# pathint/RankCompV3.jl

Hardware: AMD Instinct MI355X
Metric: gene-pair·sample comparisons/sec at 20k genes × 1k samples (higher is better)
Workload: dtype u16

## Files before the change

rankcompv3.jl_amd/_ffi.py:

```python
from __future__ import annotations

import ctypes
import os
import subprocess
from typing import NamedTuple

import numpy as np

_HERE = os.path.dirname(os.path.abspath(__file__))
LIB_PATH = os.environ.get("REO_LIB_PATH") or os.path.join(_HERE, "libreo_hip.so")
CSRC = os.path.join(_HERE, "csrc")

REO_OK, REO_EINVAL, REO_EHIP, REO_ECOMM, REO_ENOMEM = 0, -1, -2, -3, -4
NTIMINGS = 12
CALL_BINS = 8192

SYMBOLS = [
    "reo_version", "reo_last_error", "reo_create", "reo_destroy", "reo_trim_memory", "reo_set_shard", "reo_set_allreduce", "reo_set_allgather",
    "reo_create_multi", "reo_comm_unique_id", "reo_comm_init_rank",
    "reo_set_matrix_f64", "reo_set_matrix_i64", "reo_set_matrix_dev_f64", "reo_set_matrix_dev_i64",
    "reo_set_matrix_f32", "reo_set_matrix_i32", "reo_set_matrix_dev_f32", "reo_set_matrix_dev_i32",
    "reo_set_matrix_rm_f64", "reo_set_matrix_rm_i64", "reo_set_matrix_rm_f32", "reo_set_matrix_rm_i32",
    "reo_set_matrix_csc_f64", "reo_set_matrix_csc_i64", "reo_set_matrix_csc_f32", "reo_set_matrix_csc_i32",
    "reo_set_groups", "reo_compute_thresholds", "reo_set_thresholds", "reo_get_thresholds", "reo_threshold",
# ... 1203 lines not shown

    def set_profiling(self, on: bool) -> None:
        check(self._L.reo_set_profiling(self._h, 1 if on else 0))

    def reset_timings(self) -> None:
        check(self._L.reo_reset_timings(self._h))

    def timings(self) -> dict:
        ms = np.zeros(NTIMINGS, dtype=np.float64)
        check(self._L.reo_get_timings(self._h, _ptr(ms), NTIMINGS))
        return {"transform_ms": ms[0], "k1_ms": ms[1], "k2_ms": ms[2], "iter_ms": ms[3], "k3_ms": max(ms[3] - ms[2], 0.0), "k2_launches": int(ms[4]),
                "k1_launches": int(ms[5]), "exchange_ms": ms[6], "pseudobulk_ms": ms[7], "k2_full_ms": ms[8],
                "k2_full_launches": int(ms[9]), "k2_delta_ms": ms[10], "set_matrix_host_wall_ms": ms[11]}

    def info(self) -> dict:
        w = np.zeros(42, dtype=np.int64)
        check(self._L.reo_get_info(self._h, _ptr(w), 42))
        v = np.zeros(28, dtype=np.int64)
        v[:] = w[:28]
        return {"G": int(v[0]), "S": int(v[1]), "Gp": int(v[2]), "table_bytes": int(v[3]), "has_ties": int(v[4]),
                "tiles_owned": int(v[5]), "tiles_total": int(v[6]), "tile_i": int(v[7]), "chunk_j": int(v[8]),
                "chunks_per_panel": int(v[9]), "unit_h": int(v[10]), "sample_slots": int(v[11]),
                "shared_group_counts": int(v[12]), "group_count_bytes": int(v[13]), "transform_in_lds": int(v[14]), "xcc_local_histograms": int(v[15]),
                "cycle_period": int(v[16]), "cycle_found_at_pass": int(v[17]), "cycle_passes_skipped": int(v[18]), "upload_link_bytes": int(v[19]),
                "eager_range_launches": int(v[20]), "rowmajor_upload": int(v[21]),
                "csc_upload": int(v[22]), "csc_nnz": int(v[23]), "resident_dtype": int(v[24]),
                "k1_slot_order": int(v[25]), "k1_half_tiles_separated": int(v[26]), "csc_device": int(v[27]),
                "k1_unslot_form": int(w[28]), "contrast_treat": int(w[29]), "k1_slot_sides": int(w[30]),
                "masked_build": int(w[31]), "k1_slot_slice": int(w[32]), "planes_on_demand": int(w[33]),
                "perm_batch": int(w[34]), "perm_kernel_us": int(w[35]),
                "top_pairs_hist_us": int(w[36]), "top_pairs_emit_us": int(w[37]),
                "top_pairs_null_batch": int(w[38]), "top_pairs_null_us": int(w[39]),
                "top_pairs_loo_words_us": int(w[40]), "top_pairs_loo_select_us": int(w[41])}
```

rankcompv3.jl_amd/csrc/api.hip:

```cpp
#include <execinfo.h>
#include <signal.h>
#include <unistd.h>

#include <ctime>
#include <algorithm>
#include <chrono>
#include <cmath>
#include <cstdarg>
#include <cstdio>
#include <cstdlib>
#include <cstring>

#include "reo_internal.h"
#include "contrast.h"
#include "masked_pairs.h"
#include "perm_null.h"
#include "sample_counts.h"
#include "upload_csc.h"

#include <mutex>
#include <unordered_map>

namespace reo {

// ... 6 lines not shown
    std::mutex mu;
    std::vector<Block> free_blocks;
    std::unordered_map<void *, size_t> live;
    size_t cached = 0, cap = size_t(16384) << 20;
    bool read_env = false;
};
Pool &pool() { static Pool *p = new Pool(); return *p; }
size_t pool_round(size_t bytes) { return bytes <= 4096 ? 4096 : (bytes + 255) & ~size_t(255); }
hipError_t raw_alloc(void **p, size_t bytes, bool pinned) { return pinned ? hipHostMalloc(p, bytes) : hipMalloc(p, bytes); }
void raw_free(void *p, bool pinned) { if (pinned) (void)hipHostFree(p); else (void)hipFree(p); }
}

namespace {
struct Handles {
    std::mutex mu;
    std::vector<std::pair<int, hipStream_t>> streams[2];
    std::vector<std::pair<int, hipEvent_t>> events[2];
};
Handles &handles() { static Handles *h = new Handles(); return *h; }
}

hipError_t handle_stream(hipStream_t *s, int kind)
{
    int dev = 0;
    (void)hipGetDevice(&dev);
    {
        Handles &H = handles();
        std::lock_guard<std::mutex> lk(H.mu);
        auto &v = H.streams[kind];
        for (size_t i = v.size(); i-- > 0;)
            if (v[i].first == dev) { *s = v[i].second; v.erase(v.begin() + static_cast<long>(i)); return hipSuccess; }
    }
    if (kind == 0) return hipStreamCreateWithFlags(s, hipStreamNonBlocking);
    int lo_pri = 0, hi_pri = 0;
    const hipError_t e = hipDeviceGetStreamPriorityRange(&lo_pri, &hi_pri);
    return e != hipSuccess ? e : hipStreamCreateWithPriority(s, hipStreamNonBlocking, hi_pri);
}

hipError_t handle_event(hipEvent_t *ev, int kind)
{
    int dev = 0;
    (void)hipGetDevice(&dev);
    {
        Handles &H = handles();
        std::lock_guard<std::mutex> lk(H.mu);
        auto &v = H.events[kind];
        for (size_t i = v.size(); i-- > 0;)
            if (v[i].first == dev) { *ev = v[i].second; v.erase(v.begin() + static_cast<long>(i)); return hipSuccess; }
    }
    return kind ? hipEventCreate(ev) : hipEventCreateWithFlags(ev, hipEventDisableTiming);
}
// ... 183 lines not shown
}

static double wall_us()
{
    timespec ts;
    clock_gettime(CLOCK_MONOTONIC, &ts);
    return ts.tv_sec * 1e6 + ts.tv_nsec * 1e-3;
}

static void drop_ref_mask(reo_ctx *c, const char *why)
{
    c->ref_slot = -1;
    c->ref_gone = why;
}

int32_t wait_or_drop_table(reo_ctx *c)
{
    const hipError_t e = stream_wait(c);
    if (e == hipSuccess) return REO_OK;
    c->built_k = -1;
    c->table_complete = false;
    drop_ref_mask(c, "a kernel queued on this context failed and the class table was dropped");
    set_error("a kernel queued on this context failed: %s (the class table was dropped: call reo_build_pairs again)", hipGetErrorString(e));
    return REO_EHIP;
}

int32_t use(reo_ctx *c)
{
    if (!c) { set_error("null context"); return REO_EINVAL; }
    REO_HIP_CHECK(hipSetDevice(c->device));
    return REO_OK;
}

// ... 266 lines not shown
    {
        Pool &P = pool();
        std::lock_guard<std::mutex> lk(P.mu);
        all.swap(P.free_blocks);
        P.cached = 0;
    }
    int dev = 0;
    const bool have_dev = hipGetDevice(&dev) == hipSuccess;
    for (const Block &b : all) {
        if (!b.pinned) (void)hipSetDevice(b.device);
        raw_free(b.p, b.pinned);
    }
    {
        Handles &H = handles();
        std::lock_guard<std::mutex> lk(H.mu);
        for (int k = 0; k < 2; ++k) {
            for (auto &st : H.streams[k]) { (void)hipSetDevice(st.first); (void)hipStreamDestroy(st.second); }
            for (auto &ev : H.events[k]) { (void)hipSetDevice(ev.first); (void)hipEventDestroy(ev.second); }
            H.streams[k].clear(); H.events[k].clear();
        }
    }
    if (have_dev) (void)hipSetDevice(dev);
    return REO_OK;
}

const char *reo_last_error(void) { return g_err.c_str(); }

int32_t reo_create(reo_ctx **out, int32_t device, uint64_t seed)
{
    if (!out) { set_error("out is null"); return REO_EINVAL; }
    *out = nullptr;
    if (getenv("REO_DEBUG_SEGV")) install_segv_backtrace();
    int ndev = 0;
    if (hipGetDeviceCount(&ndev) != hipSuccess || ndev == 0) {
// ... 25 lines not shown
    {
        int n = 0;
        if (hipDeviceGetAttribute(&n, hipDeviceAttributeMultiprocessorCount, c->device) == hipSuccess && n > 0) c->n_cus = n;
    }
    if (const char *e = getenv("REO_SPIN_WAIT")) c->spin_wait = (e[0] != '0');
    if (const char *e = getenv("REO_CHECK_HOOK_TABLE")) c->check_hook_table = (e[0] != '0');
    if (const char *e = getenv("REO_SHARE_GROUP_COUNTS")) c->share_counts = (e[0] != '0');
    if (const char *e = getenv("REO_LIGHT_BAND")) c->light_band = std::max(0, atoi(e));
    if (const char *e = getenv("REO_HIST_BELOW")) c->hist_below = std::max(0, atoi(e));
    if (const char *e = getenv("REO_CYCLE")) c->cycle_watch = atoi(e) != 0;
    if (const char *e = getenv("REO_LIGHT")) c->light_mode = e[0] == '0' ? 0 : (e[0] == '2' ? 2 : (e[0] == '3' ? 3 : 1));
    c->light_window = light_window(); c->light_min_g = light_min_genes();
    if (const char *e = getenv("REO_LIGHT_WINDOW")) c->light_window = std::max(1, std::min(31, atoi(e)));
    if (const char *e = getenv("REO_LIGHT_MIN_G")) c->light_min_g = std::max(64, atoi(e));
    if (const char *e = getenv("REO_STATE_MIRROR")) c->state_mirror_wanted = (e[0] != '0');
    if (const char *e = getenv("REO_EXCHANGE_WAVES")) c->x_waves = std::max(1, std::min(8, atoi(e)));
    if (const char *e = getenv("REO_EAGER_UPLOAD")) c->eager_mode = std::max(0, std::min(2, atoi(e)));
    if (const char *e = getenv("REO_EAGER_CHUNK")) c->eager_chunk = std::max(1, atoi(e));
    if (const char *e = getenv("REO_EAGER_GATE")) c->eager_gate = atoi(e) != 0;
    if (const char *e = getenv("REO_EAGER_RANGES")) c->eager_ranges = std::max(1, std::min(6, atoi(e)));
    if (const char *e = getenv("REO_UPLOAD_THREADS")) c->upload_threads = std::max(0, std::min(64, atoi(e)));
    c->debug_passes = getenv("REO_DEBUG_PASSES") != nullptr;
    c->debug_stamps = getenv("REO_DEBUG_STAMPS") != nullptr;
    c->k1_stamps = getenv("REO_K1_STAMPS") != nullptr;
    hipError_t e = handle_stream(&c->stream, 0);
    if (e != hipSuccess) { delete c; set_error("hipStreamCreate failed: %s", hipGetErrorString(e)); return REO_EHIP; }
    int ok = 0;
    const char *xe = getenv("REO_XCC_LOCAL");
    if (!(xe && xe[0] == '0')) {
        const int32_t rc = xcc_selftest(c, &ok);
// ... 2 lines not shown
    c->xcc_local = ok;
    *out = c;
    return REO_OK;
}

void reo_destroy(reo_ctx *c)
{
    if (!c) return;
    for (reo_ctx *p : c->peers) reo_destroy(p);
    c->peers.clear();
    (void)hipSetDevice(c->device);
    for (int q = 0; q < 2; ++q) if (c->k1s[q]) (void)hipStreamSynchronize(c->k1s[q]);
    if (c->xs) (void)hipStreamSynchronize(c->xs);
    if (c->up) (void)hipStreamSynchronize(c->up);
    if (c->rk) (void)hipStreamSynchronize(c->rk);
    (void)hipStreamSynchronize(c->stream);
    comm_release(c);
    collect_timings(c);
    tl_release_synced = true;
    for (auto &t : c->pool) { release_event(t.a, 1); release_event(t.b, 1); }
    c->dX_owned.release(); c->pos.release(); c->lo.release(); c->hi.release(); c->goff_dev.release();
    c->table.release();
    c->t_kin.release(); c->t_kout.release(); c->t_vin.release(); c->t_vout.release(); c->t_temp.release();
    c->t_order.release(); c->t_flags.release(); c->t_slots.release(); c->unit_map.release();
    for (auto &il : c->k1_wave_items) il.buf.release();
    for (int q = 0; q < 2; ++q) { release_stream(c->k1s[q], 0); release_event(c->ev_k1_join[q], 0); }
    release_stream(c->xs, 0);
    release_stream(c->up, 0);
    release_stream(c->rk, 1);
    for (auto &e : c->ev_rk) release_event(e, 0);
// ... 7 lines not shown
    }
    release_event(c->ev_fork, 0);
    release_event(c->ev_x, 0);
    for (auto &e : c->ev_k1) release_event(e, 0);
    c->t_pos16.release(); c->t_lo16.release(); c->t_hi16.release(); c->gcounts.release();
    c->k1_slot_part.release(); c->k1_slot_maps.release(); c->pos_s.release(); c->lo_s.release(); c->k1_queue_ctr.release();
    c->t_pos32.release(); c->t_lo32.release(); c->t_hi32.release(); c->t_vin32.release(); c->t_vout32.release();
    for (int t = 0; t < 2; ++t) { c->refbits[t].release(); c->refbytes[t].release(); }
    c->raw.release(); c->delta_list.release(); c->cont.release(); c->result.release(); c->sorted_d.release(); c->sorted_p.release();
    c->rank_s.release(); c->rank_a.release(); c->scal.release(); c->blockmin.release();
    c->state.release(); c->trace.release(); c->modes.release(); c->cand.release(); c->hist.release(); c->mrank.release(); c->lstate.release(); c->clist.release(); c->olist.release(); c->units_all.release(); c->xsend.release(); c->xrecv.release(); c->check_flag.release(); c->gridbar.release(); c->chunk_v.release(); c->chunk_i.release(); c->part.release();
    if (c->host_state) pool_free(c->host_state, sizeof(IterState), true);
    if (c->host_flags) pool_free(c->host_flags, 8 * sizeof(int32_t), true);
    release_event(c->ev_flags, 0);
    if (c->host_ref) pool_free(c->host_ref, c->host_ref_cap, true);
    release_stream(c->stream, 0);
    delete c;
    tl_release_synced = false;
}

int32_t reo_set_shard(reo_ctx *c, int32_t rank, int32_t world)
{
    if (!c) { set_error("null context"); return REO_EINVAL; }
    if (world < 1 || rank < 0 || rank >= world) { set_error("bad shard %d of %d", rank, world); return REO_EINVAL; }
    if (!c->peers.empty()) { set_error("a multi-GPU context (reo_create_multi) shards by itself"); return REO_EINVAL; }
    c->rank = rank; c->world = world;
    c->built_k = -1;
    drop_ref_mask(c, "reo_set_shard dropped the class table that the last reo_identify_degs ran on");
    c->eager_k1 = false;
    c->gc_valid = false;
// ... 578 lines not shown
        st.nref = nref;
        st.nref_prev = nref;
        st.delta_cnt[0] = st.delta_cnt[1] = 0x7FFFFFFF;
        st.need_full = 1;
        st.raw_pass = -1;
        st.kstar = -1;
        st.cyc_period = -1;
        *c->host_state = st;
    }
    const bool watch = c->cycle_watch && c->light_mode != 0 && (c->light_mode == 1 || G > 65535) && G >= c->light_min_g && n_iter > 0;
    if (watch) {
        if ((rc = c->snap.ensure(2 * static_cast<size_t>(c->Gp)))) return rc;
        c->host_state->cyc_period = 0;
    }
    c->it_cycle_period = 0; c->it_cycle_at = 0; c->it_cycle_skipped = 0;
    DrainOnExit drain(c);
    if ((rc = launch_iter_init(c, c->host_ref, c->host_state))) return rc;
    c->it_pval_deg = pval_deg; c->it_padj_deg = padj_deg; c->it_n_iter = n_iter; c->it_n_conv = n_conv;
    c->it_a0 = static_cast<int>(a - 1); c->it_b0 = static_cast<int>(b - 1);
    c->k2_idx = 0;
    const int light_form = (G > 65535 && c->light_mode != 0) ? 1 : c->light_mode;
    c->it_light_form = light_form;
    c->state_mirror = light_form != 2 && c->state_mirror_wanted;
    bool small = G < c->light_min_g || c->light_mode == 0;
    c->it_no_light = false;
    int passes = 0, seen_need_full = 1, light_batches = 0, idle_light = 0, idle_any = 0;
    while (n_iter > 0) {
        const int remaining = n_iter - passes;
        const double w_loop = c->debug_passes ? wall_us() : 0.0;
        const int nfull = small ? std::min(8, remaining) : (seen_need_full ? std::min(passes == 0 ? 4 : 2, remaining) : 0);
        const int nlight = (small || seen_need_full) ? 0 : std::min(light_batches == 0 ? 32 : kLightBatch, remaining);
        if (nlight > 0) ++light_batches;
        tic(c, 3);
        for (int t = 0; t < nfull; ++t)
            if ((rc = launch_full_pass(c, false))) return rc;
        if (nlight > 0 && light_form == 2) {
            if ((rc = launch_light_persistent(c))) return rc;
        } else if (nlight > 0) {
            if ((rc = launch_light_batch(c, nlight))) return rc;
        }
        toc(c);
        if (!c->state_mirror) REO_HIP_CHECK(hipMemcpyAsync(c->host_state, c->state.p, sizeof(IterState), hipMemcpyDeviceToHost, c->stream));
        const double w0 = c->debug_passes ? wall_us() : 0.0;
        if ((rc = wait_or_drop_table(c))) return rc;
        if (c->debug_passes) fprintf(stderr, "  waited %.0f us for the batch (enqueueing it took %.0f us)\n", wall_us() - w0, w0 - w_loop);
        if (c->debug_passes && nlight > 0 && light_form == 3) {
            static LightState hs;
            if (hipMemcpy(&hs, c->lstate.p, sizeof hs, hipMemcpyDeviceToHost) == hipSuccess)
                for (int q = 1; q <= nlight; ++q)
                    if (hs.slot[q].pad0[0] || q <= 3)
                        fprintf(stderr, "  launch %d: why %d (1 window, 2 se left the bracket, 4 the histogram's cut left the band, 8 a list overflowed, 16 too many listed, 32 cut below the band), "
                                "cut of the m_lo histogram %d, listed %d, surely inside %d, cut %d (band around %d), eta %.3g, se %.10g\n", q, hs.slot[q].pad0[0], hs.slot[q].pad0[1],
                                hs.slot[q].pad0[2], hs.slot[q].pad0[3], hs.slot[q].pad0[4], hs.slot[q - 1].rec.kstar, hs.slot[q - 1].eta, hs.slot[q].se_base);
        }
// ... 6 lines not shown
        if (idle_any >= 4) {
            set_error("the iteration made no progress in four batches of launches (passes %d, need_full %d): loop control fault", passes, c->host_state->need_full);
            return REO_EHIP;
        }
        if (nlight > 0) idle_light = c->host_state->passes == passes ? idle_light + 1 : 0;
        if (idle_light >= 2 && !small) {
            small = true;
            c->it_no_light = true;
        }
        if (c->host_state->passes < passes || c->host_state->passes > n_iter) {
            set_error("the iteration's pass counter reads %d after %d of %d passes: loop control fault", c->host_state->passes, passes, n_iter);
            return REO_EHIP;
        }
        passes = c->host_state->passes;
        seen_need_full = c->host_state->need_full;
        if (c->host_state->done || passes >= n_iter) break;
        if (c->host_state->cyc_period > 0) {
            const int p = c->host_state->cyc_period, P = (p & 1) ? 2 * p : p;
            const int skip = (n_iter - passes - 1) / P * P;
            if ((rc = launch_cycle_skip(c, skip, p))) return rc;
            c->it_cycle_period = p; c->it_cycle_at = passes; c->it_cycle_skipped = skip;
            if (c->debug_passes) fprintf(stderr, "cycle: the reference set in front of pass %d equals that of pass %d; %d passes skipped\n", passes, passes - p, skip);
            passes += skip;
        }
    }
    if (passes > 0 && !c->host_state->last_full) {
        tic(c, 3);
        if ((rc = launch_full_pass(c, true))) return rc;
        toc(c);
    }
    if (trace && passes > 0)
        REO_HIP_CHECK(hipMemcpyAsync(trace, c->trace.p, sizeof(int32_t) * 2 * passes, hipMemcpyDeviceToHost, c->stream));
    const int nk2 = std::min<int>(c->k2_idx, static_cast<int>(c->modes.n));
    if (c->profiling && nk2 > 0) {
        c->k2_modes.assign(c->k2_idx, 0);
        REO_HIP_CHECK(hipMemcpyAsync(c->k2_modes.data(), c->modes.p, sizeof(int32_t) * nk2, hipMemcpyDeviceToHost, c->stream));
    }
    if (c->debug_stamps) {
        unsigned long long st[24];
        REO_HIP_CHECK(hipMemcpy(st, c->scal.p + 32, sizeof st, hipMemcpyDeviceToHost));
        if (light_form == 3) {
            fprintf(stderr, "stamps kl_one (inputs back, se, cut, lists + mask step, changed rows, delta1, sums + windows, end):");
            for (int k = 0; k <= 7; ++k) fprintf(stderr, " %lld", (long long)(st[k] - st[8]));
        } else if (light_form == 2) {
            fprintf(stderr, "stamps kl_persist, one pass (phase 1, barrier, phase 2, barrier, loads asked, cut, mask step):");
            for (int k = 1; k <= 7; ++k) fprintf(stderr, " %lld", (long long)(st[k] - st[0]));
        } else {
            fprintf(stderr, "stamps kl_head (inputs back, cut, mask step, changed rows, delta1, window flags, block sums, end):");
            for (int k = 0; k <= 7; ++k) fprintf(stderr, " %lld", (long long)(st[k] - st[8]));
            fprintf(stderr, "\nstamps kl_rank (inputs back, selection + se, p + BH rank, end):");
            for (int k = 20; k <= 23; ++k) fprintf(stderr, " %lld", (long long)(st[k] - st[19]));
        }
        fprintf(stderr, "  (x 10 ns)\n");
    }
    if (iters_run) *iters_run = passes;
    const double w_copy = c->debug_passes ? wall_us() : 0.0;
    REO_HIP_CHECK(hipMemcpyAsync(result, c->result.p, sizeof(double) * 15 * G, hipMemcpyDeviceToHost, c->stream));
    const double w_copied = c->debug_passes ? wall_us() : 0.0;
    if ((rc = wait_or_drop_table(c))) return rc;
    drain.dismiss();
    if (c->debug_passes) fprintf(stderr, "  result copy: enqueued in %.0f us, waited %.0f us\n", w_copied - w_copy, wall_us() - w_copied);
    collect_timings(c);
    if ((rc = pass_fault(c))) return rc;
    if (passes > 0) c->ref_slot = (passes - 1) & 1;
    else drop_ref_mask(c, "the last reo_identify_degs was called with n_iter <= 0: no pass ran, no tallies were counted");
    return REO_OK;
}

int32_t reo_get_ref_mask(reo_ctx *c, uint8_t *ref_mask, int32_t *nref)
{
    int32_t rc = use(c);
    if (rc) return rc;
    if (!ref_mask) { set_error("reo_get_ref_mask: ref_mask must not be null"); return REO_EINVAL; }
    if (c->ref_slot < 0 || c->built_k < 0) {
        set_error("reo_get_ref_mask: no reference set to deliver: %s", c->ref_slot < 0 ? c->ref_gone : "the class table was dropped");
// ... 222 lines not shown
{
    if (!c || !ms) { set_error("null argument"); return REO_EINVAL; }
    collect_timings(c);
    for (int i = 0; i < n && i < REO_NTIMINGS; ++i) ms[i] = c->t_ms[i];
    return REO_OK;
}

int32_t reo_get_info(reo_ctx *c, int64_t *info, int32_t n)
{
    if (!c || !info) { set_error("null argument"); return REO_EINVAL; }
    int64_t separated = 0;
    if (n > 26 && c->last_k1_slots) {
        int32_t rc = use(c);
        if (rc || (rc = launch_slot_separated(c, &separated))) return rc;
    }
    const int64_t v[42] = {c->G, c->S, c->Gp, static_cast<int64_t>(c->table.n * sizeof(uint32_t)), c->has_ties,
                           c->tiles_owned, c->tiles_total, kTileI, c->k1_cj, c->k1_q, kUnitH,
                           c->goff32.empty() ? 0 : c->goff32.back(), c->last_k1_shared,
                           static_cast<int64_t>(c->gcounts.n * sizeof(uint16_t)), c->transform_in_lds, c->xcc_local,
                           c->it_cycle_period, c->it_cycle_at, c->it_cycle_skipped, c->narrowed_bytes, c->eager_range_launches, c->rowmajor_upload,
                           c->csc_upload, c->csc_nnz, c->dtype, c->last_k1_slots, separated, c->csc_device,
                           c->last_k1_slots ? c->last_k1_unslot : 0, c->built_k >= 0 ? c->built_treat : -1,
                           c->last_k1_slots ? c->last_k1_slot_sides : 0, (c->built_k >= 0 && c->built_masked) ? 1 : 0,
                           c->last_k1_slots ? c->last_k1_slot_slice : 0, c->transformed ? c->planes_on_demand : 0, c->perm_batch, c->perm_kernel_us,
                           c->top_hist_us, c->top_emit_us, c->top_null_batch, c->top_null_us, c->top_loo_words_us, c->top_loo_select_us};
    for (int i = 0; i < n && i < 42; ++i) info[i] = v[i];
    return REO_OK;
}

}
```

rankcompv3.jl_amd/csrc/kernels.hip:

```cpp
#include <algorithm>
#include <chrono>
#include <cstddef>
#include <cstdio>
#include <cstdlib>
#include <cstring>
#include <mutex>
#include <type_traits>

#include "reo_internal.h"
#include "k1_items.h"
#include "k1_slots.h"
#include "k1_queue.h"
#include "contrast.h"
#include "tie_coin.h"

namespace reo {

namespace {

template <bool COH, class T>
__device__ __forceinline__ T ldc(const T *p)
{
    if (COH) return __hip_atomic_load(p, __ATOMIC_RELAXED, __HIP_MEMORY_SCOPE_AGENT);
    return *p;
// ... 1538 lines not shown
    int32_t *trace; int32_t *modes;
    double *cand;
    int32_t *hist;
    int hist_stride;
    int32_t *mrank;
    int replay;
    int k2_idx;
    int xcc_local;
    int32_t *olist;
    int hist_below;
    uint8_t *snap;
    int32_t *clist; int band;
    int window, light_min_g;
    unsigned long long *stamps;
    IterState *host_st;
};

#ifdef REO_STAMPS
#define STAMP(a, k) do { if (blockIdx.x == 0 && threadIdx.x == 0) (a).stamps[k] = __builtin_amdgcn_s_memrealtime(); } while (0)
#else
#define STAMP(a, k) do { } while (0)
#endif

__device__ __forceinline__ void raise_fault(const IterArgs &a, int code)
{
    a.st->fault = code;
    if (a.host_st) a.host_st->fault = code;
}

constexpr int kCandMax = 64;
constexpr int kWindow = 24;
constexpr int kLightMinG = 4096;

__device__ __forceinline__ bool full_pass_active(const IterArgs &a, int &t, int &nref)
{
    const IterState *st = a.st;
    if (a.replay) { t = st->passes - 1; nref = st->nref_prev; return t >= 0; }
    t = st->passes; nref = st->nref;
    return !st->done && st->passes < a.n_iter && st->need_full;
}

__global__ __launch_bounds__(256) void k2_tally(IterArgs a)
{
    int t, nref;
    if (!full_pass_active(a, t, nref) || a.st->raw_pass == t) return;
    const int cur = t & 1;
    const int n = a.st->delta_cnt[cur];
    const bool full = n > kDeltaMax;
    if (a.modes && blockIdx.x == 0 && threadIdx.x == 0) a.modes[a.k2_idx] = full ? 1 : 0;
    if (full) tally_rows(reinterpret_cast<const uint4 *>(a.table), reinterpret_cast<const uint4 *>(a.refbits[cur]), a.G, a.Wp / 4, a.raw);
    else if (static_cast<int>(blockIdx.x) * 256 < a.G) delta_genes(a.table, a.G, a.Wp, a.delta_list + static_cast<size_t>(cur) * a.Gp, n, a.raw);
}
// ... 875 lines not shown
#pragma unroll
        for (int q = 0; q < 4; ++q) win[q] = ps->wnext[q];
    } else {
#pragma unroll
        for (int q = 0; q < 4; ++q) win[q] = a.scal[1 + q];
    }
    if (!TAIL) STAMP(a, 0);
    int n = 0;
    bool inref = false;
    bool stepped = false;
    if (b == 0) {
        const IterState *st = a.st;
        r.t = st->passes; r.nref = st->nref; r.nref_prev = st->nref_prev; r.done = st->done; r.need_full = st->need_full;
        r.raw_pass = st->raw_pass; r.ran = 0; r.dcnt = st->delta_cnt[r.t & 1]; r.kstar = -1;
        r.cper = st->cyc_period; r.cpow = st->cyc_pow; r.clam = st->cyc_lam; r.csel = st->cyc_sel; cdiff = st->cyc_ndiff;
        r.active = (!r.done && r.t < a.n_iter && !r.need_full) ? 1 : 0;
        if (r.active) {
            n = r.raw_pass == r.t ? 0 : min(r.dcnt, kDeltaMax);
            if (static_cast<int>(threadIdx.x) < n) dl[threadIdx.x] = a.delta_list[static_cast<size_t>(r.t & 1) * Gp + threadIdx.x];
            inref = i < G && a.refbytes[r.t & 1][i] != 0;
            lds_barrier();
        }
    } else if (r.active && bfail) {
        r.active = 0; r.need_full = 1;
    } else if (r.active && cfound) {
        r.active = 0; r.cper = cfound;
    } else if (r.active) {
        const int t = r.t, cur = t & 1, nxt = cur ^ 1;
        const int off = hist_first(r.kstar, a.hist_below), srel = sig - off;
        {
            const int32_t *hist = a.hist + static_cast<size_t>(pb) * kHistParts * a.hist_stride;
// ... 147 lines not shown
            st->i_iter = r.t - (r.done ? 1 : 0);
            st->raw_pass = r.raw_pass;
            st->delta_cnt[r.t & 1] = r.dcnt;
            if (r.ran) st->last_full = 0;
            if (stepped) { a.scal[1] = win[0]; a.scal[2] = win[1]; a.scal[3] = win[2]; a.scal[4] = win[3]; }
            if (a.host_st) {
                IterState *h = a.host_st;
                h->passes = r.t; h->done = r.done; h->need_full = r.need_full; h->delta_cnt[r.t & 1] = r.dcnt;
                h->cyc_period = r.cper;
                if (r.ran) h->last_full = 0;
            }
        }
        return;
    }
    if (r.active) r.raw_pass = r.t;
    if (blockIdx.x == 0 && threadIdx.x == 0) ls->slot[b].rec = r;
    if (!r.active || static_cast<int>(blockIdx.x) * 256 >= G) {
        if (blockIdx.x == 0 && wave == 0) { cyc_close(); if (lane == 0) { ls->slot[b].cdiff = cdiff; ls->slot[b].cfound = cfound; } }
        return;
    }
    const int pbuf = b & 1;
    LightCnt *lc = &ls->slot[b].lc;
    const double wa_lo = win[0], wa_hi = win[1], wb_lo = win[2], wb_hi = win[3];
    double v = 0.0;
    bool inner = false, inA = false, inB = false, belowA = false, belowB = false;
    if (n) {
        int d[kRaw];
        delta_counts_block(a.table, a.Wp, dl, n, d, dbuf);
        if (!TAIL) STAMP(a, 3);
        if (i < G) {
            r0.x += d[0]; r0.y += d[1]; r0.z += d[2]; r0.w += d[3];
// ... 1520 lines not shown
    for (int t = 0; t < 2; ++t) { a.refbits[t] = c->refbits[t].p; a.refbytes[t] = c->refbytes[t].p; }
    a.raw = c->raw.p; a.delta_list = c->delta_list.p; a.result = c->result.p;
    const int nchunk = (a.G + kSortChunk - 1) / kSortChunk;
    a.chunk_v = c->chunk_v.p; a.chunk_i = c->chunk_i.p;
    a.chunk_spl = c->chunk_v.p + static_cast<size_t>(nchunk) * kSortChunk;
    a.sorted_d = c->sorted_d.p; a.sorted_spl = c->sorted_d.p + ((c->G + 63) / 64) * 64;
    a.sorted_p = c->sorted_p.p; a.rank_s = c->rank_s.p; a.rank_a = c->rank_a.p;
    a.part = c->part.p; a.blockmin = c->blockmin.p; a.scal = c->scal.p;
    a.trace = c->trace.p; a.modes = nullptr;
    a.cand = c->cand.p; a.hist = c->hist.p; a.hist_stride = static_cast<int>(c->hist.n / (3 * kHistParts)); a.mrank = c->mrank.p;
    a.replay = replay; a.k2_idx = 0;
    a.clist = c->clist.p; a.olist = c->olist.p; a.band = c->light_band; a.hist_below = c->hist_below; a.snap = c->snap.p; a.xcc_local = c->xcc_local;
    a.window = c->light_window; a.light_min_g = (c->it_no_light || c->light_mode == 0) ? 0x7FFFFFFF : c->light_min_g;
    a.stamps = reinterpret_cast<unsigned long long *>(c->scal.p + 32);
    a.host_st = c->state_mirror ? c->host_state : nullptr;
    return a;
}

int32_t launch_full_pass(reo_ctx *c, bool replay)
{
    IterArgs a = iter_args(c, replay ? 1 : 0);
    const int G = a.G, nb = (G + 255) / 256;
    const int nchunk = (G + kSortChunk - 1) / kSortChunk;
    const int nmerge = (nchunk * kSortChunk + kMergeThreads / kMergeLanes - 1) / (kMergeThreads / kMergeLanes);
    if (!replay) {
        if (c->k2_idx < static_cast<int>(c->modes.n)) { a.modes = c->modes.p; a.k2_idx = c->k2_idx; }
        ++c->k2_idx;
        tic(c, 2);
        k2_tally<<<(G + 3) / 4, 256, 0, c->stream>>>(a);
        toc(c);
        c->t_ms[4] += 1.0;
    }
    k3_derive<<<nb, 256, 0, c->stream>>>(a);
    k3_sort_chunks<<<nchunk, kSortChunk, 0, c->stream>>>(a);
    const size_t spl_bytes = static_cast<size_t>(nchunk) * kSplit * sizeof(double);
    if (spl_bytes > (size_t(48) << 10))
        REO_HIP_CHECK(hipFuncSetAttribute(reinterpret_cast<const void *>(k3_merge_rank), hipFuncAttributeMaxDynamicSharedMemorySize, static_cast<int>(spl_bytes)));
    k3_merge_rank<<<nmerge, kMergeThreads, spl_bytes, c->stream>>>(a, nchunk);
    k3_abs_rank<<<nb, 256, static_cast<size_t>((G + 63) / 64) * sizeof(double), c->stream>>>(a, nmerge);
    k3_bh_local<<<(G + 1023) / 1024, 1024, 0, c->stream>>>(a);
    k3_finalize<<<c->Gp / 256, 256, 0, c->stream>>>(a);
    REO_HIP_CHECK(hipGetLastError());
    return REO_OK;
}

int32_t launch_light_persistent(reo_ctx *c)
{
    const IterArgs a = iter_args(c, 0);
    const unsigned nwg = static_cast<unsigned>(a.Gp / 256);
    REO_HIP_CHECK(hipMemsetAsync(c->gridbar.p, 0, sizeof(unsigned), c->stream));
    REO_HIP_CHECK(hipMemsetAsync(c->lstate.p, 0, 2 * sizeof(LightSlot), c->stream));
    kl_persist<<<nwg, 256, 0, c->stream>>>(a, c->lstate.p, c->gridbar.p);
    REO_HIP_CHECK(hipGetLastError());
    return REO_OK;
}

int32_t launch_light_batch(reo_ctx *c, int nlight)
{
    const IterArgs a = iter_args(c, 0);
    const int nb = (a.G + 255) / 256, nbp = a.Gp / 256;
    if (nlight < 1 || nlight > kLightBatch) { set_error("light batch of %d passes", nlight); return REO_EINVAL; }
    REO_HIP_CHECK(hipMemsetAsync(c->lstate.p, 0, static_cast<size_t>(nlight + 1) * sizeof(LightSlot), c->stream));
    if (c->it_light_form == 3) {
        REO_HIP_CHECK(hipMemsetAsync(c->hist.p, 0, static_cast<size_t>(kHistParts) * a.hist_stride * sizeof(int32_t), c->stream));
        for (int b = 0; b < nlight; ++b) kl_one<false><<<nbp, 256, 0, c->stream>>>(a, c->lstate.p, b);
        kl_one<true><<<nbp, 256, 0, c->stream>>>(a, c->lstate.p, nlight);
        REO_HIP_CHECK(hipGetLastError());
        return REO_OK;
    }
    for (int b = 0; b < nlight; ++b) {
        if (b < 2) kl_head<false, false><<<nbp, 256, 0, c->stream>>>(a, c->lstate.p, b);
        else kl_head<false, true><<<nbp, 256, 0, c->stream>>>(a, c->lstate.p, b);
        kl_rank<<<nb, 256, 0, c->stream>>>(a, c->lstate.p, b);
    }
    if (nlight < 2) kl_head<true, false><<<nbp, 256, 0, c->stream>>>(a, c->lstate.p, nlight);
    else kl_head<true, true><<<nbp, 256, 0, c->stream>>>(a, c->lstate.p, nlight);
    REO_HIP_CHECK(hipGetLastError());
    return REO_OK;
}

int32_t xcc_selftest(reo_ctx *c, int *ok)
{
    *ok = 0;
    DevBuf<int32_t> buf;
    static std::mutex mu;
    static int verdict[64];
    {
// ... 39 lines not shown
```

rankcompv3.jl_amd/csrc/reo_internal.h:

```cpp
#pragma once

#include <hip/hip_runtime.h>

#include <cstdint>
#include <functional>
#include <string>
#include <vector>

#include "reo_hip.h"

namespace reo {

constexpr int kTileJ = 256;
constexpr int kTileI = 32;
constexpr int kPlanes = 4;
constexpr int kUnitH = 32;
constexpr int kRJ = 4;
constexpr int kRJTies = 2;
constexpr int kMaxGenes = 262143;
constexpr int kGenePad = 1024;
constexpr int kRaw = 8;
constexpr int kDeltaMax = 128;
constexpr int kSortChunk = 1024;

// ... 296 lines not shown
    int light_window = 24, light_min_g = 4096;
    int light_mode = 1;
    reo::DevBuf<int32_t> olist;
    reo::DevBuf<int32_t> hist, mrank;
    double it_pval_deg = 1.0, it_padj_deg = 0.05;
    int it_n_iter = 0, it_n_conv = 0, it_a0 = 0, it_b0 = 0;
    int k2_idx = 0;
    int it_light_form = 1;
    bool it_no_light = false;
    reo::IterState *host_state = nullptr;
    bool state_mirror_wanted = true;
    bool debug_passes = false, debug_stamps = false, k1_stamps = false;
    bool state_mirror = false;
    uint8_t *host_ref = nullptr;
    size_t host_ref_cap = 0;

    bool profiling = false;
    double t_ms[REO_NTIMINGS] = {0};
    std::vector<std::pair<int, reo::StageTimer>> pending;
    std::vector<reo::StageTimer> pool;
    std::vector<size_t> open;
    std::vector<int32_t> k2_modes;
    size_t k2_seen = 0;
};

namespace reo {

int32_t run_transform(reo_ctx *c);
int32_t ensure_planes(reo_ctx *c);
enum { kLayoutColMajor = 0, kLayoutRowMajor = 1, kLayoutCsc = 2 };
// ... 10 lines not shown
int32_t launch_k1(reo_ctx *c, int k, int sides = 3, bool keep_table = false, const int32_t *gate = nullptr, const K1Range *range = nullptr,
                  bool prepare = false, int treat = -1);
int32_t k1_planes_fit(reo_ctx *c, bool *fit, size_t *need_bytes);
int64_t exchange_unit_words(const reo_ctx *c);
int32_t exchange_units_per_rank(const reo_ctx *c);
int32_t launch_pack_units(reo_ctx *c, int m0 = 0, int mcnt = -1, uint32_t *send = nullptr, hipStream_t st = nullptr);
int32_t launch_expand_units(reo_ctx *c, int m0 = 0, int mcnt = -1, const uint32_t *recv = nullptr, hipStream_t st = nullptr);
int32_t launch_slot_separated(reo_ctx *c, int64_t *half_tiles);
int32_t launch_counts(reo_ctx *c, int64_t i0, int64_t i1, int64_t j0, int64_t j1, uint16_t *d_gt, uint16_t *d_eq);
int32_t launch_check_table(reo_ctx *c, int *bad);
int32_t launch_decode(reo_ctx *c, int64_t i0, int64_t i1, int64_t j0, int64_t j1, uint8_t *d_code);
int32_t launch_pack_ref(reo_ctx *c, const uint8_t *d_bytes, uint32_t *d_bits);
int32_t launch_cycle_skip(reo_ctx *c, int skip, int period);
int32_t launch_iter_init(reo_ctx *c, const uint8_t *host_ref, const IterState *host_state);
int32_t launch_tally(reo_ctx *c, int nref);
int32_t launch_full_pass(reo_ctx *c, bool replay);
int32_t launch_light_persistent(reo_ctx *c);
int32_t launch_light_batch(reo_ctx *c, int nlight);
int32_t xcc_selftest(reo_ctx *c, int *ok);
int32_t light_min_genes();
int32_t light_window();
int32_t launch_mccullagh(reo_ctx *c, const int32_t *d_cont, int64_t n, double *d_out);

int32_t launch_pair_count(reo_ctx *c, const int32_t *d_genes, int64_t n_genes, const uint32_t *d_maskbits, uint32_t class_mask, int32_t *d_count);
int32_t launch_pair_fill(reo_ctx *c, const int32_t *d_genes, int64_t n_genes, const uint32_t *d_maskbits, uint32_t class_mask, const int64_t *d_rowptr,
                         int32_t *d_partner, uint8_t *d_code, int64_t capacity, int32_t *d_flag);

int plane_bits(int64_t G);
int32_t launch_sample_counts(reo_ctx *c, const int32_t *d_genes, int64_t n_queries, const uint32_t *d_maskbits, uint32_t class_mask,
                             const int32_t *d_slot2col, int32_t *d_sel, int32_t *d_gt, int32_t *d_eq);

int32_t launch_sample_fisher(reo_ctx *c, int64_t n_queries, const int32_t *d_sel_a, const int32_t *d_sel_b, const int32_t *d_gt_a,
                             const int32_t *d_eq_a, const int32_t *d_gt_b, const int32_t *d_eq_b, const double *d_lf, int64_t lf_entries,
// ... 48 lines not shown

int32_t comm_allgather(reo_ctx *c, const void *send, void *recv, int64_t bytes_per_rank, hipStream_t st = nullptr);
void comm_release(reo_ctx *c);
void comm_abort(reo_ctx *c);
int32_t comm_wait(reo_ctx *c);
int32_t multi_build_pairs(reo_ctx *lead, int32_t k, int32_t (*build_local)(reo_ctx *, int32_t));

void tic(reo_ctx *c, int slot);
void toc(reo_ctx *c);
void collect_timings(reo_ctx *c);

int32_t use(reo_ctx *c);
int32_t no_multi(reo_ctx *c, const char *what);
int32_t need_complete_table(reo_ctx *c);
int32_t ensure_transform(reo_ctx *c);
int32_t wait_or_drop_table(reo_ctx *c);
bool mask_in_force(reo_ctx *c);
int32_t refuse_under_mask(reo_ctx *c, const char *what);
int32_t upload_slot2col(reo_ctx *c, const std::vector<int32_t> &map);
struct DrainOnExit {
    reo_ctx *c;
    bool armed = true;
    explicit DrainOnExit(reo_ctx *ctx) : c(ctx) {}
    DrainOnExit(const DrainOnExit &) = delete;
    DrainOnExit &operator=(const DrainOnExit &) = delete;
    void dismiss() { armed = false; }
    ~DrainOnExit()
    {
        if (!armed || !c || !c->stream) return;
        (void)hipStreamSynchronize(c->stream);
    }
};

}
```

Baseline: 52420 billion.

## Chain light-pass batches via mid-batch host mark and queue replay ahead

```diff
diff --git a/rankcompv3.jl_amd/_ffi.py b/rankcompv3.jl_amd/_ffi.py
--- a/rankcompv3.jl_amd/_ffi.py
+++ b/rankcompv3.jl_amd/_ffi.py
@@ -1241,8 +1241,8 @@
                 "k2_full_launches": int(ms[9]), "k2_delta_ms": ms[10], "set_matrix_host_wall_ms": ms[11]}
 
     def info(self) -> dict:
-        w = np.zeros(42, dtype=np.int64)
-        check(self._L.reo_get_info(self._h, _ptr(w), 42))
+        w = np.zeros(46, dtype=np.int64)
+        check(self._L.reo_get_info(self._h, _ptr(w), 46))
         v = np.zeros(28, dtype=np.int64)
         v[:] = w[:28]
         return {"G": int(v[0]), "S": int(v[1]), "Gp": int(v[2]), "table_bytes": int(v[3]), "has_ties": int(v[4]),
@@ -1258,4 +1258,6 @@
                 "perm_batch": int(w[34]), "perm_kernel_us": int(w[35]),
                 "top_pairs_hist_us": int(w[36]), "top_pairs_emit_us": int(w[37]),
                 "top_pairs_null_batch": int(w[38]), "top_pairs_null_us": int(w[39]),
-                "top_pairs_loo_words_us": int(w[40]), "top_pairs_loo_select_us": int(w[41])}
+                "top_pairs_loo_words_us": int(w[40]), "top_pairs_loo_select_us": int(w[41]),
+                "chain_batches": int(w[42]), "chain_batches_idle": int(w[43]),
+                "chain_replays_ahead": int(w[44]), "chain_replays_ahead_idle": int(w[45])}
diff --git a/rankcompv3.jl_amd/csrc/api.hip b/rankcompv3.jl_amd/csrc/api.hip
--- a/rankcompv3.jl_amd/csrc/api.hip
+++ b/rankcompv3.jl_amd/csrc/api.hip
@@ -44,7 +44,7 @@
 namespace {
 struct Handles {
     std::mutex mu;
-    std::vector<std::pair<int, hipStream_t>> streams[2];
+    std::vector<std::pair<int, hipStream_t>> streams[3];
     std::vector<std::pair<int, hipEvent_t>> events[2];
 };
 Handles &handles() { static Handles *h = new Handles(); return *h; }
@@ -64,7 +64,7 @@
     if (kind == 0) return hipStreamCreateWithFlags(s, hipStreamNonBlocking);
     int lo_pri = 0, hi_pri = 0;
     const hipError_t e = hipDeviceGetStreamPriorityRange(&lo_pri, &hi_pri);
-    return e != hipSuccess ? e : hipStreamCreateWithPriority(s, hipStreamNonBlocking, hi_pri);
+    return e != hipSuccess ? e : hipStreamCreateWithPriority(s, hipStreamNonBlocking, kind == 1 ? hi_pri : lo_pri);
 }
 
 hipError_t handle_event(hipEvent_t *ev, int kind)
@@ -278,9 +278,9 @@
     c->ref_gone = why;
 }
 
-int32_t wait_or_drop_table(reo_ctx *c)
-{
-    const hipError_t e = stream_wait(c);
+int32_t wait_or_drop_table(reo_ctx *c, hipEvent_t mark)
+{
+    const hipError_t e = mark ? hipEventSynchronize(mark) : stream_wait(c);
     if (e == hipSuccess) return REO_OK;
     c->built_k = -1;
     c->table_complete = false;
@@ -577,10 +577,13 @@
     {
         Handles &H = handles();
         std::lock_guard<std::mutex> lk(H.mu);
+        for (int k = 0; k < 3; ++k) {
+            for (auto &st : H.streams[k]) { (void)hipSetDevice(st.first); (void)hipStreamDestroy(st.second); }
+            H.streams[k].clear();
+        }
         for (int k = 0; k < 2; ++k) {
-            for (auto &st : H.streams[k]) { (void)hipSetDevice(st.first); (void)hipStreamDestroy(st.second); }
             for (auto &ev : H.events[k]) { (void)hipSetDevice(ev.first); (void)hipEventDestroy(ev.second); }
-            H.streams[k].clear(); H.events[k].clear();
+            H.events[k].clear();
         }
     }
     if (have_dev) (void)hipSetDevice(dev);
@@ -636,6 +639,10 @@
     if (const char *e = getenv("REO_LIGHT_WINDOW")) c->light_window = std::max(1, std::min(31, atoi(e)));
     if (const char *e = getenv("REO_LIGHT_MIN_G")) c->light_min_g = std::max(64, atoi(e));
     if (const char *e = getenv("REO_STATE_MIRROR")) c->state_mirror_wanted = (e[0] != '0');
+    if (const char *e = getenv("REO_CHAIN")) c->chain = (e[0] != '0');
+    if (const char *e = getenv("REO_CHAIN_AHEAD")) c->chain_ahead = std::max(1, std::min(kLightBatch, atoi(e)));
+    if (const char *e = getenv("REO_LIGHT_BATCH_FIRST")) c->light_batch_first = std::max(1, std::min(kLightBatchFirst, atoi(e)));
+    if (const char *e = getenv("REO_LIGHT_BATCH")) c->light_batch = std::max(1, std::min(kLightBatch, atoi(e)));
     if (const char *e = getenv("REO_EXCHANGE_WAVES")) c->x_waves = std::max(1, std::min(8, atoi(e)));
     if (const char *e = getenv("REO_EAGER_UPLOAD")) c->eager_mode = std::max(0, std::min(2, atoi(e)));
     if (const char *e = getenv("REO_EAGER_CHUNK")) c->eager_chunk = std::max(1, atoi(e));
@@ -668,6 +675,7 @@
     if (c->xs) (void)hipStreamSynchronize(c->xs);
     if (c->up) (void)hipStreamSynchronize(c->up);
     if (c->rk) (void)hipStreamSynchronize(c->rk);
+    if (c->rs) (void)hipStreamSynchronize(c->rs);
     (void)hipStreamSynchronize(c->stream);
     comm_release(c);
     collect_timings(c);
@@ -705,6 +713,10 @@
     if (c->host_flags) pool_free(c->host_flags, 8 * sizeof(int32_t), true);
     release_event(c->ev_flags, 0);
     if (c->host_ref) pool_free(c->host_ref, c->host_ref_cap, true);
+    if (c->host_trace) pool_free(c->host_trace, c->host_trace_cap, true);
+    release_event(c->ev_mark, 0);
+    release_event(c->ev_derive, 0);
+    release_stream(c->rs, 2);
     release_stream(c->stream, 0);
     delete c;
     tl_release_synced = false;
@@ -1313,6 +1325,17 @@
         c->host_state->cyc_period = 0;
     }
     c->it_cycle_period = 0; c->it_cycle_at = 0; c->it_cycle_skipped = 0;
+    if (c->chain && !c->ev_mark) REO_HIP_CHECK(handle_event(&c->ev_mark, 0));
+    const size_t trace_ints = 2 * static_cast<size_t>(n_iter > 0 ? n_iter : 1);
+    const size_t trace_bytes = sizeof(int32_t) * (trace_ints + c->modes.n);
+    if (c->chain && !c->rs) REO_HIP_CHECK(handle_stream(&c->rs, 2));
+    if (c->chain && !c->ev_derive) REO_HIP_CHECK(handle_event(&c->ev_derive, 0));
+    if (c->chain && c->host_trace_cap < trace_bytes) {
+        if (c->host_trace) pool_free(c->host_trace, c->host_trace_cap, true);
+        c->host_trace = nullptr; c->host_trace_cap = 0;
+        REO_HIP_CHECK(pool_alloc(reinterpret_cast<void **>(&c->host_trace), trace_bytes, true));
+        c->host_trace_cap = trace_bytes;
+    }
     DrainOnExit drain(c);
     if ((rc = launch_iter_init(c, c->host_ref, c->host_state))) return rc;
     c->it_pval_deg = pval_deg; c->it_padj_deg = padj_deg; c->it_n_iter = n_iter; c->it_n_conv = n_conv;
@@ -1324,19 +1347,62 @@
     bool small = G < c->light_min_g || c->light_mode == 0;
     c->it_no_light = false;
     int passes = 0, seen_need_full = 1, light_batches = 0, idle_light = 0, idle_any = 0;
+    bool ahead = false;
+    const size_t Gs = static_cast<size_t>(G);
+    auto queue_replay_and_copies = [&](size_t ints_of_trace) -> int32_t {
+        const std::function<int32_t()> mark_derive = [&]() -> int32_t {
+            REO_HIP_CHECK(hipEventRecord(c->ev_derive, c->stream));
+            REO_HIP_CHECK(hipStreamWaitEvent(c->rs, c->ev_derive, 0));
+            return REO_OK;
+        };
+        int32_t r = launch_full_pass(c, true, &mark_derive);
+        if (r) return r;
+        if (trace) REO_HIP_CHECK(hipMemcpyAsync(c->host_trace, c->trace.p, sizeof(int32_t) * ints_of_trace, hipMemcpyDeviceToHost, c->stream));
+        const size_t nmodes = std::min(static_cast<size_t>(c->k2_idx), c->modes.n);
+        if (c->profiling && nmodes > 0)
+            REO_HIP_CHECK(hipMemcpyAsync(c->host_trace + trace_ints, c->modes.p, sizeof(int32_t) * nmodes, hipMemcpyDeviceToHost, c->stream));
+        REO_HIP_CHECK(hipMemcpyAsync(result + 2 * Gs, c->result.p + 2 * Gs, sizeof(double) * 13 * Gs, hipMemcpyDeviceToHost, c->rs));
+        REO_HIP_CHECK(hipMemcpyAsync(result, c->result.p, sizeof(double) * 2 * Gs, hipMemcpyDeviceToHost, c->stream));
+        return REO_OK;
+    };
     while (n_iter > 0) {
         const int remaining = n_iter - passes;
         const double w_loop = c->debug_passes ? wall_us() : 0.0;
-        const int nfull = small ? std::min(8, remaining) : (seen_need_full ? std::min(passes == 0 ? 4 : 2, remaining) : 0);
-        const int nlight = (small || seen_need_full) ? 0 : std::min(light_batches == 0 ? 32 : kLightBatch, remaining);
+        int nfull = 0, nlight = 0;
+        chain_batch(small, seen_need_full != 0, passes, light_batches, remaining, c->light_batch_first, c->light_batch, &nfull, &nlight);
         if (nlight > 0) ++light_batches;
+        ahead = false;
+        int chained_from = -1;
         tic(c, 3);
         for (int t = 0; t < nfull; ++t)
             if ((rc = launch_full_pass(c, false))) return rc;
         if (nlight > 0 && light_form == 2) {
             if ((rc = launch_light_persistent(c))) return rc;
         } else if (nlight > 0) {
-            if ((rc = launch_light_batch(c, nlight))) return rc;
+            int queued = passes;
+            for (int nl = nlight;;) {
+                const int mark_b = chain_mark_launch(c->chain, light_form, c->state_mirror, nl, c->chain_ahead);
+                if ((rc = launch_light_batch(c, nl, mark_b))) return rc;
+                const int start = queued;
+                queued += nl;
+                if (mark_b < 0) break;
+                if ((rc = wait_or_drop_table(c, c->ev_mark))) return rc;
+                const ChainMark m = {c->host_state->passes, c->host_state->done, c->host_state->need_full, c->host_state->cyc_period, c->host_state->fault};
+                const ChainStep step = chain_decide(m, start, mark_b, queued, n_iter);
+                if (c->debug_passes) fprintf(stderr, "  mark of a batch of %d light launches: passes %d, done %d, need_full %d, period %d -> %s\n", nl, m.passes, m.done, m.need_full,
+                                             m.cyc_period, step == kChainLight ? "the next batch is queued" : (step == kChainReplay ? "the replay is queued" : "wait"));
+                if (step == kChainWait) break;
+                if (step == kChainReplay) {
+                    if ((rc = queue_replay_and_copies(2 * static_cast<size_t>(n_iter)))) return rc;
+                    ahead = true;
+                    ++c->chain_replays;
+                    break;
+                }
+                nl = std::min(c->light_batch, n_iter - queued);
+                ++light_batches;
+                ++c->chain_batches;
+                chained_from = queued;
+            }
         }
         toc(c);
         if (!c->state_mirror) REO_HIP_CHECK(hipMemcpyAsync(c->host_state, c->state.p, sizeof(IterState), hipMemcpyDeviceToHost, c->stream));
@@ -1373,7 +1439,12 @@
         }
         passes = c->host_state->passes;
         seen_need_full = c->host_state->need_full;
+        if (chained_from >= 0 && passes <= chained_from) ++c->chain_idle;
         if (c->host_state->done || passes >= n_iter) break;
+        if (ahead) {
+            ++c->chain_replays_idle;
+            REO_HIP_CHECK(hipStreamSynchronize(c->rs));
+        }
         if (c->host_state->cyc_period > 0) {
             const int p = c->host_state->cyc_period, P = (p & 1) ? 2 * p : p;
             const int skip = (n_iter - passes - 1) / P * P;
@@ -1383,17 +1454,26 @@
             passes += skip;
         }
     }
-    if (passes > 0 && !c->host_state->last_full) {
+    const bool want_replay = !ahead && passes > 0 && !c->host_state->last_full;
+    const int nk2 = std::min<int>(c->k2_idx, static_cast<int>(c->modes.n));
+    bool staged = ahead;
+    if (want_replay && c->chain) {
         tic(c, 3);
-        if ((rc = launch_full_pass(c, true))) return rc;
+        if ((rc = queue_replay_and_copies(2 * static_cast<size_t>(passes)))) return rc;
         toc(c);
-    }
-    if (trace && passes > 0)
-        REO_HIP_CHECK(hipMemcpyAsync(trace, c->trace.p, sizeof(int32_t) * 2 * passes, hipMemcpyDeviceToHost, c->stream));
-    const int nk2 = std::min<int>(c->k2_idx, static_cast<int>(c->modes.n));
-    if (c->profiling && nk2 > 0) {
-        c->k2_modes.assign(c->k2_idx, 0);
-        REO_HIP_CHECK(hipMemcpyAsync(c->k2_modes.data(), c->modes.p, sizeof(int32_t) * nk2, hipMemcpyDeviceToHost, c->stream));
+        staged = true;
+    } else if (!ahead) {
+        if (want_replay) {
+            tic(c, 3);
+            if ((rc = launch_full_pass(c, true))) return rc;
+            toc(c);
+        }
+        if (trace && passes > 0)
+            REO_HIP_CHECK(hipMemcpyAsync(c->chain ? c->host_trace : trace, c->trace.p, sizeof(int32_t) * 2 * passes, hipMemcpyDeviceToHost, c->stream));
+        if (c->profiling && nk2 > 0) {
+            if (!c->chain) c->k2_modes.assign(c->k2_idx, 0);
+            REO_HIP_CHECK(hipMemcpyAsync(c->chain ? c->host_trace + trace_ints : c->k2_modes.data(), c->modes.p, sizeof(int32_t) * nk2, hipMemcpyDeviceToHost, c->stream));
+        }
     }
     if (c->debug_stamps) {
         unsigned long long st[24];
@@ -1414,10 +1494,16 @@
     }
     if (iters_run) *iters_run = passes;
     const double w_copy = c->debug_passes ? wall_us() : 0.0;
-    REO_HIP_CHECK(hipMemcpyAsync(result, c->result.p, sizeof(double) * 15 * G, hipMemcpyDeviceToHost, c->stream));
+    if (!staged) REO_HIP_CHECK(hipMemcpyAsync(result, c->result.p, sizeof(double) * 15 * G, hipMemcpyDeviceToHost, c->stream));
     const double w_copied = c->debug_passes ? wall_us() : 0.0;
     if ((rc = wait_or_drop_table(c))) return rc;
+    if (staged) REO_HIP_CHECK(hipStreamSynchronize(c->rs));
     drain.dismiss();
+    if (c->chain && trace && passes > 0) memcpy(trace, c->host_trace, sizeof(int32_t) * 2 * passes);
+    if (c->chain && c->profiling && nk2 > 0) {
+        c->k2_modes.assign(c->k2_idx, 0);
+        std::copy(c->host_trace + trace_ints, c->host_trace + trace_ints + nk2, c->k2_modes.begin());
+    }
     if (c->debug_passes) fprintf(stderr, "  result copy: enqueued in %.0f us, waited %.0f us\n", w_copied - w_copy, wall_us() - w_copied);
     collect_timings(c);
     if ((rc = pass_fault(c))) return rc;
@@ -1670,7 +1756,7 @@
         int32_t rc = use(c);
         if (rc || (rc = launch_slot_separated(c, &separated))) return rc;
     }
-    const int64_t v[42] = {c->G, c->S, c->Gp, static_cast<int64_t>(c->table.n * sizeof(uint32_t)), c->has_ties,
+    const int64_t v[46] = {c->G, c->S, c->Gp, static_cast<int64_t>(c->table.n * sizeof(uint32_t)), c->has_ties,
                            c->tiles_owned, c->tiles_total, kTileI, c->k1_cj, c->k1_q, kUnitH,
                            c->goff32.empty() ? 0 : c->goff32.back(), c->last_k1_shared,
                            static_cast<int64_t>(c->gcounts.n * sizeof(uint16_t)), c->transform_in_lds, c->xcc_local,
@@ -1679,9 +1765,10 @@
                            c->last_k1_slots ? c->last_k1_unslot : 0, c->built_k >= 0 ? c->built_treat : -1,
                            c->last_k1_slots ? c->last_k1_slot_sides : 0, (c->built_k >= 0 && c->built_masked) ? 1 : 0,
                            c->last_k1_slots ? c->last_k1_slot_slice : 0, c->transformed ? c->planes_on_demand : 0, c->perm_batch, c->perm_kernel_us,
-                           c->top_hist_us, c->top_emit_us, c->top_null_batch, c->top_null_us, c->top_loo_words_us, c->top_loo_select_us};
-    for (int i = 0; i < n && i < 42; ++i) info[i] = v[i];
-    return REO_OK;
-}
-
-}
+                           c->top_hist_us, c->top_emit_us, c->top_null_batch, c->top_null_us, c->top_loo_words_us, c->top_loo_select_us,
+                           c->chain_batches, c->chain_idle, c->chain_replays, c->chain_replays_idle};
+    for (int i = 0; i < n && i < 46; ++i) info[i] = v[i];
+    return REO_OK;
+}
+
+}
diff --git a/rankcompv3.jl_amd/csrc/chain_policy.h b/rankcompv3.jl_amd/csrc/chain_policy.h
--- /dev/null
+++ b/rankcompv3.jl_amd/csrc/chain_policy.h
@@ -0,0 +1,33 @@
+#pragma once
+#include <cstdint>
+
+namespace reo {
+
+constexpr int kChainAhead = 6;
+constexpr int kLightBatchFirst = 32;
+
+enum ChainStep { kChainWait = 0, kChainLight = 1, kChainReplay = 2 };
+
+struct ChainMark { int32_t passes, done, need_full, cyc_period, fault; };
+
+inline void chain_batch(bool small, bool need_full, int passes, int light_batches, int remaining, int first, int later, int *nfull, int *nlight)
+{
+    const int cap = light_batches == 0 ? first : later;
+    *nfull = small ? (remaining < 8 ? remaining : 8) : (need_full ? (remaining < (passes == 0 ? 4 : 2) ? remaining : (passes == 0 ? 4 : 2)) : 0);
+    *nlight = (small || need_full) ? 0 : (remaining < cap ? remaining : cap);
+}
+
+inline int chain_mark_launch(bool chain, int light_form, bool mirror, int nlight, int ahead)
+{
+    return (chain && light_form == 1 && mirror && ahead >= 1 && nlight > ahead) ? nlight - ahead : -1;
+}
+
+inline ChainStep chain_decide(const ChainMark &m, int start, int mark_b, int queued, int n_iter)
+{
+    if (mark_b < 0) return kChainWait;
+    const bool alive = !m.done && !m.need_full && m.cyc_period <= 0 && !m.fault && m.passes == start + mark_b && m.passes < n_iter;
+    if (!alive) return kChainWait;
+    return queued >= n_iter ? kChainReplay : kChainLight;
+}
+
+}
diff --git a/rankcompv3.jl_amd/csrc/kernels.hip b/rankcompv3.jl_amd/csrc/kernels.hip
--- a/rankcompv3.jl_amd/csrc/kernels.hip
+++ b/rankcompv3.jl_amd/csrc/kernels.hip
@@ -1576,6 +1576,7 @@
     int window, light_min_g;
     unsigned long long *stamps;
     IterState *host_st;
+    int mark_b;
 };
 
 #ifdef REO_STAMPS
@@ -1597,7 +1598,7 @@
 __device__ __forceinline__ bool full_pass_active(const IterArgs &a, int &t, int &nref)
 {
     const IterState *st = a.st;
-    if (a.replay) { t = st->passes - 1; nref = st->nref_prev; return t >= 0; }
+    if (a.replay) { t = st->passes - 1; nref = st->nref_prev; return t >= 0 && (st->done || st->passes >= a.n_iter) && !st->last_full; }
     t = st->passes; nref = st->nref;
     return !st->done && st->passes < a.n_iter && st->need_full;
 }
@@ -2503,7 +2504,7 @@
         r.t = st->passes; r.nref = st->nref; r.nref_prev = st->nref_prev; r.done = st->done; r.need_full = st->need_full;
         r.raw_pass = st->raw_pass; r.ran = 0; r.dcnt = st->delta_cnt[r.t & 1]; r.kstar = -1;
         r.cper = st->cyc_period; r.cpow = st->cyc_pow; r.clam = st->cyc_lam; r.csel = st->cyc_sel; cdiff = st->cyc_ndiff;
-        r.active = (!r.done && r.t < a.n_iter && !r.need_full) ? 1 : 0;
+        r.active = (!r.done && r.t < a.n_iter && !r.need_full && r.cper <= 0 && st->fault == 0) ? 1 : 0;
         if (r.active) {
             n = r.raw_pass == r.t ? 0 : min(r.dcnt, kDeltaMax);
             if (static_cast<int>(threadIdx.x) < n) dl[threadIdx.x] = a.delta_list[static_cast<size_t>(r.t & 1) * Gp + threadIdx.x];
@@ -2681,7 +2682,14 @@
         return;
     }
     if (r.active) r.raw_pass = r.t;
-    if (blockIdx.x == 0 && threadIdx.x == 0) ls->slot[b].rec = r;
+    if (blockIdx.x == 0 && threadIdx.x == 0) {
+        ls->slot[b].rec = r;
+        if (b == a.mark_b && a.host_st) {
+            IterState *h = a.host_st;
+            h->passes = r.t; h->done = r.done; h->need_full = r.need_full; h->delta_cnt[r.t & 1] = r.dcnt;
+            h->cyc_period = r.cper;
+        }
+    }
     if (!r.active || static_cast<int>(blockIdx.x) * 256 >= G) {
         if (blockIdx.x == 0 && wave == 0) { cyc_close(); if (lane == 0) { ls->slot[b].cdiff = cdiff; ls->slot[b].cfound = cfound; } }
         return;
@@ -4232,10 +4240,11 @@
     a.window = c->light_window; a.light_min_g = (c->it_no_light || c->light_mode == 0) ? 0x7FFFFFFF : c->light_min_g;
     a.stamps = reinterpret_cast<unsigned long long *>(c->scal.p + 32);
     a.host_st = c->state_mirror ? c->host_state : nullptr;
+    a.mark_b = -1;
     return a;
 }
 
-int32_t launch_full_pass(reo_ctx *c, bool replay)
+int32_t launch_full_pass(reo_ctx *c, bool replay, const std::function<int32_t()> *behind_derive)
 {
     IterArgs a = iter_args(c, replay ? 1 : 0);
     const int G = a.G, nb = (G + 255) / 256;
@@ -4250,6 +4259,10 @@
         c->t_ms[4] += 1.0;
     }
     k3_derive<<<nb, 256, 0, c->stream>>>(a);
+    if (behind_derive) {
+        const int32_t rc = (*behind_derive)();
+        if (rc) return rc;
+    }
     k3_sort_chunks<<<nchunk, kSortChunk, 0, c->stream>>>(a);
     const size_t spl_bytes = static_cast<size_t>(nchunk) * kSplit * sizeof(double);
     if (spl_bytes > (size_t(48) << 10))
@@ -4273,11 +4286,13 @@
     return REO_OK;
 }
 
-int32_t launch_light_batch(reo_ctx *c, int nlight)
-{
-    const IterArgs a = iter_args(c, 0);
+int32_t launch_light_batch(reo_ctx *c, int nlight, int mark_b)
+{
+    IterArgs a = iter_args(c, 0);
     const int nb = (a.G + 255) / 256, nbp = a.Gp / 256;
     if (nlight < 1 || nlight > kLightBatch) { set_error("light batch of %d passes", nlight); return REO_EINVAL; }
+    if (mark_b >= 0 && (mark_b >= nlight || c->it_light_form != 1 || !a.host_st || !c->ev_mark)) { set_error("light batch of %d passes: mark at launch %d", nlight, mark_b); return REO_EINVAL; }
+    a.mark_b = mark_b;
     REO_HIP_CHECK(hipMemsetAsync(c->lstate.p, 0, static_cast<size_t>(nlight + 1) * sizeof(LightSlot), c->stream));
     if (c->it_light_form == 3) {
         REO_HIP_CHECK(hipMemsetAsync(c->hist.p, 0, static_cast<size_t>(kHistParts) * a.hist_stride * sizeof(int32_t), c->stream));
@@ -4289,6 +4304,7 @@
     for (int b = 0; b < nlight; ++b) {
         if (b < 2) kl_head<false, false><<<nbp, 256, 0, c->stream>>>(a, c->lstate.p, b);
         else kl_head<false, true><<<nbp, 256, 0, c->stream>>>(a, c->lstate.p, b);
+        if (b == mark_b) REO_HIP_CHECK(hipEventRecord(c->ev_mark, c->stream));
         kl_rank<<<nb, 256, 0, c->stream>>>(a, c->lstate.p, b);
     }
     if (nlight < 2) kl_head<true, false><<<nbp, 256, 0, c->stream>>>(a, c->lstate.p, nlight);
diff --git a/rankcompv3.jl_amd/csrc/reo_internal.h b/rankcompv3.jl_amd/csrc/reo_internal.h
--- a/rankcompv3.jl_amd/csrc/reo_internal.h
+++ b/rankcompv3.jl_amd/csrc/reo_internal.h
@@ -8,6 +8,7 @@
 #include <vector>
 
 #include "reo_hip.h"
+#include "chain_policy.h"
 
 namespace reo {
 
@@ -334,6 +335,15 @@
     bool state_mirror = false;
     uint8_t *host_ref = nullptr;
     size_t host_ref_cap = 0;
+    bool chain = true;
+    int chain_ahead = reo::kChainAhead;
+    int light_batch_first = reo::kLightBatchFirst, light_batch = reo::kLightBatch;
+    hipEvent_t ev_mark = nullptr;
+    int32_t *host_trace = nullptr;
+    size_t host_trace_cap = 0;
+    hipStream_t rs = nullptr;
+    hipEvent_t ev_derive = nullptr;
+    int64_t chain_batches = 0, chain_idle = 0, chain_replays = 0, chain_replays_idle = 0;
 
     bool profiling = false;
     double t_ms[REO_NTIMINGS] = {0};
@@ -374,9 +384,9 @@
 int32_t launch_cycle_skip(reo_ctx *c, int skip, int period);
 int32_t launch_iter_init(reo_ctx *c, const uint8_t *host_ref, const IterState *host_state);
 int32_t launch_tally(reo_ctx *c, int nref);
-int32_t launch_full_pass(reo_ctx *c, bool replay);
+int32_t launch_full_pass(reo_ctx *c, bool replay, const std::function<int32_t()> *behind_derive = nullptr);
 int32_t launch_light_persistent(reo_ctx *c);
-int32_t launch_light_batch(reo_ctx *c, int nlight);
+int32_t launch_light_batch(reo_ctx *c, int nlight, int mark_b = -1);
 int32_t xcc_selftest(reo_ctx *c, int *ok);
 int32_t light_min_genes();
 int32_t light_window();
@@ -455,7 +465,7 @@
 int32_t no_multi(reo_ctx *c, const char *what);
 int32_t need_complete_table(reo_ctx *c);
 int32_t ensure_transform(reo_ctx *c);
-int32_t wait_or_drop_table(reo_ctx *c);
+int32_t wait_or_drop_table(reo_ctx *c, hipEvent_t mark = nullptr);
 bool mask_in_force(reo_ctx *c);
 int32_t refuse_under_mask(reo_ctx *c, const char *what);
 int32_t upload_slot2col(reo_ctx *c, const std::vector<int32_t> &map);
@@ -469,6 +479,7 @@
     ~DrainOnExit()
     {
         if (!armed || !c || !c->stream) return;
+        if (c->rs) (void)hipStreamSynchronize(c->rs);
         (void)hipStreamSynchronize(c->stream);
     }
 };
```

New measurement: 51740 billion. -1.3%, worse.
